# opentrack/neuralnet-tracker-traincode

Hardware: AMD Instinct MI355X
Metric: face-crops/sec fwd+bwd @ batch 512 (higher is better)
Workload: dtype f32; 1 GPU; NetworkWithPointHead(mobilenetv1, point head on, NLL off = training-script defaults): zero_grad + fwd + multi-task loss + bwd + fused clip/Adam step; per_gpu_batch=512, global_batch=512, input=129x129x1 f32, parallelism=dp1

## Files before the change

### neuralnet-tracker-traincode_amd/csrc/pwconv_r.hip

```cpp
#include "ttk_common.h"
#include "conv_geom.h"
#include "split16.h"
#include <type_traits>


namespace ttk {

enum { RMODE_FWD = 0, RMODE_DGRAD = 1 };
template <int N, typename F, int I = 0>
__device__ __forceinline__ void static_for(F&& f) {
  if constexpr (I < N) {
    f(std::integral_constant<int, I>{});
    static_for<N, F, I + 1>(static_cast<F&&>(f));
  }
}
__device__ __forceinline__ f32x16 rmfma(f16x8 a, f16x8 b, f32x16 c) { return __builtin_amdgcn_mfma_f32_32x32x16_f16(a, b, c, 0, 0, 0); }
constexpr int kRBN = 256;

__device__ __forceinline__ void rbarrier() {
  asm volatile("s_waitcnt lgkmcnt(0)" ::: "memory");
  __builtin_amdgcn_s_barrier();
  asm volatile("" ::: "memory");
}

__device__ __forceinline__ unsigned rlow2(unsigned h, float x0, float x1) {
  unsigned l;
  asm("v_fma_mixlo_f16 %0, %1, -1.0, %2 op_sel_hi:[1,0,0]\n\t"
      "v_fma_mixhi_f16 %0, %1, -1.0, %3 op_sel:[1,0,0] op_sel_hi:[1,0,0]"
      : "=&v"(l)
      : "v"(h), "v"(x0), "v"(x1));
  return l;
}
__device__ __forceinline__ __amdgpu_buffer_rsrc_t rbuf(const float* base) {
  return __builtin_amdgcn_make_buffer_rsrc(const_cast<float*>(base), 0, 0x7fffffff, 0x00020000);
}
__device__ __forceinline__ f32x4 rbuf_ld4(__amdgpu_buffer_rsrc_t r, unsigned elem_off) {
  return __builtin_bit_cast(f32x4, __builtin_amdgcn_raw_buffer_load_b128(r, elem_off * 4u, 0, 2));
}

template <int RBLK>
struct RGeo {
  static constexpr int RB = 32 * RBLK;
  static constexpr int WM = RBLK == 8 ? 4 : 2, WN = 8 / WM;
  static constexpr int TM = RBLK / WM, TN = 8 / WN;
  static constexpr int APL = RB * 32, BPL = kRBN * 32;
  static constexpr int kStage = 2 * APL + 2 * BPL;
  static constexpr int kStr = kStage + 64;
  static constexpr int kRing = 2 * 2 * kStr;
  static constexpr int CH = 32 * WM;
  static constexpr int LDC = kRBN + 4;
  static constexpr int kEpi = CH * LDC * 4 + 12 * 2 * kRBN * 4;
  static constexpr int kCst = 4 * 1024 * 4;
  static constexpr int kSmem = kRing + kCst > kEpi ? kRing + kCst : kEpi;
};

template <int RBLK, int MODE, int NW, typename Acc, bool M16 = false>
__device__ __forceinline__ void r_epilogue(unsigned char* lds, Acc& acc, float* __restrict__ out, const float* __restrict__ E0, const float* __restrict__ bnE,
                                           float* __restrict__ part, int64_t M, int Nout, int64_t m0, int64_t m_end, int n0, unsigned by, float sa, float sb) {
  using G = RGeo<RBLK>;
  constexpr int WM = G::WM, WN = G::WN, TM = G::TM, TN = G::TN;
  constexpr bool FWD = MODE == RMODE_FWD;
  const int tid = threadIdx.x;
  const int wave = __builtin_amdgcn_readfirstlane(tid >> 6);
  constexpr int LDC = G::LDC, CH = G::CH;
  float* Cs = reinterpret_cast<float*>(lds);
  float* red = reinterpret_cast<float*>(lds + CH * LDC * 4);
  const int hw_ = tid >> 5, c4 = (hw_ & 7) * 8 + (tid & 7), rg = (hw_ >> 3) * 4 + ((tid >> 3) & 3);
  const int col = n0 + 4 * c4;
  const float inv = 1.f / (sa * sb);
  float4 esc = f4(0.f), emean = f4(0.f), ebeta = f4(0.f);
  if constexpr (!FWD) {
    esc = ld4(bnE + TTK_BN_SCALE * Nout + col); emean = ld4(bnE + TTK_BN_MEAN * Nout + col); ebeta = ld4(bnE + TTK_BN_BETA * Nout + col);
  } else {
    if (bnE) emean = ld4(bnE + col);
  }
  float4 s1 = f4(0.f), s2 = f4(0.f);
  constexpr int NRG = NW == 12 ? 6 : 8, NGRP = (CH + NW * NRG - 1) / (NW * NRG);
  float4 ev[2][NRG];
  auto tile_row = [&](int c, int cr) -> int64_t { return m0 + (cr >> 5) * (32 * TM) + c * 32 + (cr & 31); };
  auto e_load = [&](auto idxc) {
    constexpr int idx = decltype(idxc)::value, c = idx / NGRP, g = idx % NGRP;
    if constexpr (!FWD && idx < TM * NGRP) {
#pragma unroll
      for (int u = 0; u < NRG; ++u) {
        const int cr = rg + NW * (g * NRG + u);
        const int64_t grow = tile_row(c, cr);
        ev[idx & 1][u] = f4(0.f);
        if (cr < CH && grow < m_end) ev[idx & 1][u] = ld4(E0 + act_off(grow, col, M));
      }
    }
  };
  static_for<TM>([&](auto cc) {
    constexpr int c = decltype(cc)::value;
    if (wave < 8) {
      const int lane = tid & 63, wm = wave / WN, wn = wave % WN, r = lane & 31, h = lane >> 5;
      if constexpr (M16) {
        const int r16 = lane & 15, g4 = lane >> 4;
#pragma unroll
        for (int s_ = 0; s_ < 2; ++s_)
#pragma unroll
          for (int j = 0; j < 2 * TN; ++j)
#pragma unroll
            for (int i = 0; i < 4; ++i) Cs[(wm * 32 + s_ * 16 + 4 * g4 + i) * LDC + wn * (32 * TN) + j * 16 + r16] = acc[2 * c + s_][j][i];
      } else {
#pragma unroll
      for (int j = 0; j < TN; ++j)
#pragma unroll
        for (int e = 0; e < 16; ++e) Cs[(wm * 32 + (e & 3) + 8 * (e >> 2) + 4 * h) * LDC + wn * (32 * TN) + j * 32 + r] = acc[c][j][e];
      }
    }
    if constexpr (c == 0) e_load(std::integral_constant<int, 0>{});
    __syncthreads();
    static_for<NGRP>([&](auto gc) {
      constexpr int g = decltype(gc)::value, idx = c * NGRP + g;
      e_load(std::integral_constant<int, idx + 1>{});
#pragma unroll
      for (int u = 0; u < NRG; ++u) {
        const int cr = rg + NW * (g * NRG + u);
        const int64_t grow = tile_row(c, cr);
        if (cr >= CH || grow >= m_end) continue;
        float4 v = ld4(Cs + cr * LDC + 4 * c4);
        v = make_float4(v.x * inv, v.y * inv, v.z * inv, v.w * inv);
        const size_t o = act_off(grow, col, M);
        if constexpr (FWD) {
          st4(out + o, v);
          v = sub4(v, emean);
          s1 = add4(s1, v);
          s2 = fma4(v, v, s2);
        } else {
          const float4 yc = sub4(ev[idx & 1][u], emean);
          v = mask4(v, fma4(esc, yc, ebeta));
          st4(out + o, v);
          s1 = add4(s1, v);
          s2 = fma4(v, yc, s2);
        }
      }
    });
    __syncthreads();
  });
  if (part) {
    st4(red + (rg * 2 + 0) * kRBN + 4 * c4, s1);
    st4(red + (rg * 2 + 1) * kRBN + 4 * c4, s2);
    __syncthreads();
    if (tid < 2 * kRBN) {
      const int which = tid / kRBN, c = tid % kRBN;
      float a = 0.f;
#pragma unroll
      for (int qq = 0; qq < NW; ++qq) a += red[(qq * 2 + which) * kRBN + c];
      part[(size_t)by * 2 * Nout + (size_t)which * Nout + n0 + c] = a;
    }
  }
}

template <int RBLK, int MODE>
__global__ void __launch_bounds__(768) pw16r_k(const float* __restrict__ A0, const float* __restrict__ A1, const float* __restrict__ bnA,
                                               const uint16_t* __restrict__ Bq, const float* __restrict__ wmax, float* __restrict__ out,
                                               const float* __restrict__ E0, const float* __restrict__ bnE, float* __restrict__ part, int64_t M,
                                               int K, int Nout, int RT) {
  using G = RGeo<RBLK>;
  constexpr int RB = G::RB, WM = G::WM, WN = G::WN, TM = G::TM, TN = G::TN, APL = G::APL, BPL = G::BPL, kStr = G::kStr;
  constexpr bool FWD = MODE == RMODE_FWD;
  __shared__ __attribute__((aligned(16))) unsigned char lds[G::kSmem];

  const int tid = threadIdx.x;
  const unsigned Gd = gridDim.x, Lid = blockIdx.x, NB = Nout / kRBN;
  const unsigned xq = Gd / 8, xr = Gd % 8, xcd = Lid % 8;
  const unsigned tile = (xcd < xr ? xcd * (xq + 1) : xr * (xq + 1) + (xcd - xr) * xq) + Lid / 8;
  const unsigned bx = tile % NB, by = tile / NB;
  const int64_t m0 = (int64_t)by * RT;
  const int64_t m_end = m0 + RT < M ? m0 + RT : M;
  const int n0 = bx * kRBN;
  const int nks = K / 32;
  const int wave = __builtin_amdgcn_readfirstlane(tid >> 6);
  const float sa = pow2_scale(bnA[(size_t)TTK_BN_AUX * K + (FWD ? TTK_AUX_ACT_BOUND : TTK_AUX_DY_BOUND)]);
  const float sb = pow2_scale(*wmax);
  f32x16 acc[TM][TN];
  float* cst = reinterpret_cast<float*>(lds + G::kRing);
  {
    constexpr int NQ = FWD ? 3 : 4;
    for (int i = tid * 4; i < NQ * K; i += 768 * 4) {
      const int j = i / K, c = i - j * K;
      const int row = FWD ? (j == 0 ? TTK_BN_SCALE : (j == 1 ? TTK_BN_MEAN : TTK_BN_BETA)) : (j == 0 ? TTK_BN_GA : (j == 1 ? TTK_BN_GMEAN : (j == 2 ? TTK_BN_GB : TTK_BN_MEAN)));
      float4 v = ld4(bnA + (size_t)row * K + c);
      if (j == 0 || j == 2) v = make_float4(v.x * sa, v.y * sa, v.z * sa, v.w * sa);
      st4(cst + i, v);
    }
    __syncthreads();
  }

  if (wave >= 8) {
    __builtin_amdgcn_s_setprio(3);
    const int pt = tid - 512;
    const int row0 = pt >> 3, kq8 = pt & 7;
    const int sub = kq8 >> 2, chunk = (kq8 >> 1) & 1, o8 = (kq8 & 1) * 8;
    constexpr int AP = RBLK;
    constexpr int GPS = FWD ? 1 : 2;
    constexpr int NSLOT = FWD ? 2 : 3;
    static_assert(AP % GPS == 0 && (GPS & (GPS - 1)) == 0, "groups per step: a power of two that divides the row passes");
    constexpr int G = AP / GPS;
    constexpr int UNR = NSLOT % GPS == 0 ? NSLOT : (GPS % NSLOT == 0 ? GPS : NSLOT * GPS);
    f32x4 ra0[NSLOT][G] = {}, ra1[NSLOT][FWD ? 1 : G] = {};
    unsigned live = 0u;
#pragma unroll
    for (int i = 0; i < AP; ++i) live |= (m0 + row0 + 32 * i < m_end ? 1u : 0u) << i;
    const unsigned aoff0 = (unsigned)(row0 * kCB + kq8 * 4);
    const float* cq = cst + kq8 * 4;
    unsigned char* wbase = lds + sub * kStr + o8;
    const int NG = nks * GPS;

    auto load_g = [&](int ks, auto hfc, auto slotc) {
      constexpr int slot = decltype(slotc)::value, hf = decltype(hfc)::value;
      const __amdgpu_buffer_rsrc_t r0 = rbuf(A0 + ((size_t)ks * act_block_stride(M) + (size_t)m0 * kCB));
      const __amdgpu_buffer_rsrc_t r1 = rbuf((FWD ? (const float*)nullptr : A1) + ((size_t)ks * act_block_stride(M) + (size_t)m0 * kCB));
#pragma unroll
      for (int u = 0; u < G; ++u) {
        const int i = hf * G + u;
        const unsigned o = ((live >> i) & 1u) ? aoff0 + (unsigned)(i * 32 * kCB) : (unsigned)(kq8 * 4);
        ra0[slot][u] = rbuf_ld4(r0, o);
        if constexpr (!FWD) ra1[slot][u] = rbuf_ld4(r1, o);
      }
    };
    auto conv_g = [&](int ks, auto hfc, auto slotc) {
      constexpr int slot = decltype(slotc)::value, hf = decltype(hfc)::value;
      unsigned char* S = wbase + (ks & 1) * 2 * kStr;
      const float* cs = cq + ks * 32;
      const f32x4 c0 = *reinterpret_cast<const f32x4*>(cs), q1 = *reinterpret_cast<const f32x4*>(cs + K), c2 = *reinterpret_cast<const f32x4*>(cs + 2 * K);
      f32x4 q3 = c2;
      if constexpr (!FWD) q3 = *reinterpret_cast<const f32x4*>(cs + 3 * K);
#pragma unroll
      for (int u = 0; u < G; ++u) {
        const int i = hf * G + u;
        f32x4 v;
        if constexpr (FWD) {
          v = c0 * (ra0[slot][u] - q1) + c2;
          v.x = fmaxf(v.x, 0.f); v.y = fmaxf(v.y, 0.f); v.z = fmaxf(v.z, 0.f); v.w = fmaxf(v.w, 0.f);
        } else {
          v = c0 * (ra0[slot][u] - q1) + c2 * (ra1[slot][u] - q3);
        }
        if (!((live >> i) & 1u)) v = f32x4{0.f, 0.f, 0.f, 0.f};
        split_store16(v, S + swz16(row0 + 32 * i, chunk), APL);
      }
    };
    static_for<NSLOT>([&](auto dc) {
      constexpr int d = decltype(dc)::value;
      if (d < NG) load_g(d / GPS, std::integral_constant<int, d % GPS>{}, dc);
    });
    for (int n0 = 0; n0 < NG; n0 += UNR) {
      static_for<UNR>([&](auto dc) {
        constexpr int d = decltype(dc)::value;
        using HF = std::integral_constant<int, d % GPS>;
        using SL = std::integral_constant<int, d % NSLOT>;
        const int n = n0 + d;
        if (n < NG) {
          conv_g(n / GPS, HF{}, SL{});
          if (n + NSLOT < NG) load_g((n + NSLOT) / GPS, std::integral_constant<int, (d + NSLOT) % GPS>{}, SL{});
          if constexpr (d % GPS == GPS - 1) {
            __builtin_amdgcn_sched_barrier(0);
            rbarrier();
          }
        }
      });
    }
    rbarrier();
  } else {
    const int lane = tid & 63, wm = wave / WN, wn = wave % WN;
    const int r = lane & 31, h = lane >> 5;
    constexpr bool HOLD_A = TM <= TN;
    constexpr int TH = HOLD_A ? TM : TN, TS = HOLD_A ? TN : TM;
    constexpr int HPL = HOLD_A ? APL : BPL, SPL = HOLD_A ? BPL : APL;
    int hold_off[TH], strm_off[TS];
#pragma unroll
    for (int x = 0; x < TH; ++x) hold_off[x] = HOLD_A ? swz16(wm * (32 * TM) + x * 32 + r, h) : 2 * APL + swz16(wn * (32 * TN) + x * 32 + r, h);
#pragma unroll
    for (int x = 0; x < TS; ++x) strm_off[x] = HOLD_A ? 2 * APL + swz16(wn * (32 * TN) + x * 32 + r, h) : swz16(wm * (32 * TM) + x * 32 + r, h);
#pragma unroll
    for (int i = 0; i < TM; ++i)
#pragma unroll
      for (int j = 0; j < TN; ++j)
#pragma unroll
        for (int e = 0; e < 16; ++e) acc[i][j][e] = 0.f;
    f16x8 hold[TH][2] = {}, strm[2][2] = {};
    const int64_t bplane = (int64_t)K * Nout;
    const uint16_t* bsrc = Bq + ((wave >> 1) & 1) * bplane + ((int64_t)(wave >> 2) * Nout + n0 + (wave & 1) * 128) * 16 + lane * 8;
    const int bdst = (wave >> 2) * kStr + 2 * APL + ((wave >> 1) & 1) * BPL + (wave & 1) * 4096;
    const unsigned lds_base = (unsigned)(size_t)(__attribute__((address_space(3))) unsigned char*)lds;
    auto dma_b = [&](int ks) {
      const uint16_t* sp = bsrc + (int64_t)ks * 2 * Nout * 16;
      const unsigned d = __builtin_amdgcn_readfirstlane(lds_base + (unsigned)((ks & 1) * 2 * kStr + bdst));
#pragma unroll
      for (int j = 0; j < 4; ++j) {
        unsigned keep;
        asm volatile("s_mov_b32 %0, m0\n\ts_mov_b32 m0, %2\n\ts_nop 0\n\tglobal_load_lds_dwordx4 %1, off\n\ts_mov_b32 m0, %0"
                     : "=&s"(keep)
                     : "v"(sp + j * 512), "s"(d + j * 1024)
                     : "memory");
      }
    };
    dma_b(0);
    asm volatile("s_waitcnt vmcnt(0)" ::: "memory");
    rbarrier();
    auto rd = [&](const unsigned char* S, int plane_bytes, int off, int p) { return *reinterpret_cast<const f16x8*>(S + p * plane_bytes + off); };
    for (int it = 0; it < nks; ++it) {
      if (it + 1 < nks) dma_b(it + 1);
      const unsigned char* S0 = lds + (it & 1) * 2 * kStr;
#pragma unroll
      for (int p = 0; p < 2; ++p) {
#pragma unroll
        for (int y = 0; y < TH; ++y) hold[y][p] = rd(S0, HPL, hold_off[y], p);
        strm[0][p] = rd(S0, SPL, strm_off[0], p);
      }
#pragma unroll
      for (int sub = 0; sub < 2; ++sub) {
        const unsigned char* S = S0 + sub * kStr;
#pragma unroll
        for (int x = 0; x < TS; ++x) {
          const int cur = (sub * TS + x) & 1;
          const bool last = x + 1 == TS;
          if (!last) {
#pragma unroll
            for (int p = 0; p < 2; ++p) strm[cur ^ 1][p] = rd(S, SPL, strm_off[x + 1], p);
          } else if (sub == 0) {
#pragma unroll
            for (int p = 0; p < 2; ++p) strm[cur ^ 1][p] = rd(S + kStr, SPL, strm_off[0], p);
          }
#pragma unroll
          for (int y = 0; y < TH; ++y) {
            if constexpr (HOLD_A) {
              acc[y][x] = rmfma(hold[y][0], strm[cur][1], acc[y][x]);
              acc[y][x] = rmfma(hold[y][1], strm[cur][0], acc[y][x]);
              acc[y][x] = rmfma(hold[y][0], strm[cur][0], acc[y][x]);
            } else {
              acc[x][y] = rmfma(strm[cur][0], hold[y][1], acc[x][y]);
              acc[x][y] = rmfma(strm[cur][1], hold[y][0], acc[x][y]);
              acc[x][y] = rmfma(strm[cur][0], hold[y][0], acc[x][y]);
            }
            if (last && sub == 0) {
#pragma unroll
              for (int p = 0; p < 2; ++p) hold[y][p] = rd(S + kStr, HPL, hold_off[y], p);
            }
          }
        }
      }
      asm volatile("s_waitcnt vmcnt(0)" ::: "memory");
      rbarrier();
    }
  }
  r_epilogue<RBLK, MODE, 12>(lds, acc, out, E0, bnE, part, M, Nout, m0, m_end, n0, by, sa, sb);
}

template <int RBLK>
struct MGeo {
  using G = RGeo<RBLK>;
  static constexpr int NW = 8;
  static constexpr int kEpi = G::CH * G::LDC * 4 + NW * 2 * kRBN * 4;
  static constexpr int kSmem = G::kRing + G::kCst > kEpi ? G::kRing + G::kCst : kEpi;
};

template <int RBLK>
__global__ void __launch_bounds__(512) pw16m_k(const float* __restrict__ A0, const float* __restrict__ A1, const float* __restrict__ bnA,
                                               const uint16_t* __restrict__ Bq, const float* __restrict__ wmax, float* __restrict__ out,
                                               const float* __restrict__ E0, const float* __restrict__ bnE, float* __restrict__ part, int64_t M,
                                               int K, int Nout, int RT) {
  using G = RGeo<RBLK>;
  constexpr int RB = G::RB, WM = G::WM, WN = G::WN, TM = G::TM, TN = G::TN, APL = G::APL, BPL = G::BPL, kStr = G::kStr;
  __shared__ __attribute__((aligned(16))) unsigned char lds[MGeo<RBLK>::kSmem];

  const int tid = threadIdx.x;
  const unsigned Gd = gridDim.x, Lid = blockIdx.x, NB = Nout / kRBN;
  const unsigned xq = Gd / 8, xr = Gd % 8, xcd = Lid % 8;
  const unsigned tile = (xcd < xr ? xcd * (xq + 1) : xr * (xq + 1) + (xcd - xr) * xq) + Lid / 8;
  const unsigned bx = tile % NB, by = tile / NB;
  const int64_t m0 = (int64_t)by * RT;
  const int64_t m_end = m0 + RT < M ? m0 + RT : M;
  const int n0 = bx * kRBN;
  const int nks = K / 32;
  const int wave = __builtin_amdgcn_readfirstlane(tid >> 6);
  const float sa = pow2_scale(bnA[(size_t)TTK_BN_AUX * K + TTK_AUX_DY_BOUND]);
  const float sb = pow2_scale(*wmax);
  f32x4 acc16[2 * TM][2 * TN];
  float* cst = reinterpret_cast<float*>(lds + G::kRing);
  {
    for (int i = tid * 4; i < 4 * K; i += 512 * 4) {
      const int j = i / K, c = i - j * K;
      const int row = j == 0 ? TTK_BN_GA : (j == 1 ? TTK_BN_GMEAN : (j == 2 ? TTK_BN_GB : TTK_BN_MEAN));
      float4 v = ld4(bnA + (size_t)row * K + c);
      if (j == 0 || j == 2) v = make_float4(v.x * sa, v.y * sa, v.z * sa, v.w * sa);
      st4(cst + i, v);
    }
    __syncthreads();
  }

  const int row0 = tid >> 3, kq8 = tid & 7;
  const int sub_ = kq8 >> 2, chunk = (kq8 >> 1) & 1, o8 = (kq8 & 1) * 8;
  constexpr int AP = RB / 64;
  constexpr int NA = AP * 2;
  f32x4 ra0[2][AP] = {}, ra1[2][AP] = {};
  unsigned live = 0u;
#pragma unroll
  for (int u = 0; u < AP; ++u) live |= (m0 + row0 + 64 * u < m_end ? 1u : 0u) << u;
  const unsigned aoff0 = (unsigned)(row0 * kCB + kq8 * 4);
  const float* cq = cst + kq8 * 4;
  unsigned char* wbase = lds + sub_ * kStr + o8 + swz16(row0, chunk);

  auto load_a = [&](int ks, auto setc) {
    constexpr int set = decltype(setc)::value;
    const __amdgpu_buffer_rsrc_t r0 = rbuf(A0 + ((size_t)ks * act_block_stride(M) + (size_t)m0 * kCB));
    const __amdgpu_buffer_rsrc_t r1 = rbuf(A1 + ((size_t)ks * act_block_stride(M) + (size_t)m0 * kCB));
#pragma unroll
    for (int u = 0; u < AP; ++u) {
      const unsigned o = ((live >> u) & 1u) ? aoff0 + (unsigned)(u * 64 * kCB) : (unsigned)(kq8 * 4);
      ra0[set][u] = rbuf_ld4(r0, o);
      ra1[set][u] = rbuf_ld4(r1, o);
    }
  };
  f32x4 cc0 = {}, cq1 = {}, cc2 = {}, cq3 = {};
  f32x4 pv = {};
  uint2 ph = make_uint2(0u, 0u);
  auto conv_consts = [&](int ks) {
    const float* cs = cq + ks * 32;
    cc0 = *reinterpret_cast<const f32x4*>(cs); cq1 = *reinterpret_cast<const f32x4*>(cs + K); cc2 = *reinterpret_cast<const f32x4*>(cs + 2 * K);
    cq3 = *reinterpret_cast<const f32x4*>(cs + 3 * K);
  };
  int conv_ks = 0;
  auto conv_part = [&](auto setc, auto slotc, auto ppc) {
    constexpr int set = decltype(setc)::value, slot = decltype(slotc)::value, pp = decltype(ppc)::value, u = pp >> 1;
    if constexpr ((pp & 1) == 0) {
      conv_consts(conv_ks);
      f32x4 v = cc0 * (ra0[set][u] - cq1) + cc2 * (ra1[set][u] - cq3);
      if (m0 + 64 * u + 63 >= m_end) {
        if (!((live >> u) & 1u)) v = f32x4{0.f, 0.f, 0.f, 0.f};
      }
      const f16x2 h01 = __builtin_convertvector(f32x2{v.x, v.y}, f16x2), h23 = __builtin_convertvector(f32x2{v.z, v.w}, f16x2);
      pv = v;
      ph = make_uint2(__builtin_bit_cast(unsigned, h01), __builtin_bit_cast(unsigned, h23));
    } else {
      const unsigned l01 = rlow2(ph.x, pv.x, pv.y), l23 = rlow2(ph.y, pv.z, pv.w);
      unsigned char* dst = wbase + slot * 2 * kStr + u * 64 * 32;
      *reinterpret_cast<uint2*>(dst) = ph;
      *reinterpret_cast<uint2*>(dst + APL) = make_uint2(l01, l23);
    }
  };

  const int lane = tid & 63, wm = wave / WN, wn = wave % WN;
  static_assert(TM * TN == RBLK && 2 * AP == RBLK, "4 RBLK MFMA triples per step, one of the 2 AP conversion parts behind every fourth");
  const int r = lane & 31, h = lane >> 5;
  constexpr bool HOLD_A = TM <= TN;
  constexpr int TH = HOLD_A ? TM : TN;
  int hold_off[TH];
#pragma unroll
  for (int x = 0; x < TH; ++x) hold_off[x] = HOLD_A ? swz16(wm * (32 * TM) + x * 32 + r, h) : 2 * APL + swz16(wn * (32 * TN) + x * 32 + r, h);
#pragma unroll
  for (int i = 0; i < 2 * TM; ++i)
#pragma unroll
    for (int j = 0; j < 2 * TN; ++j) acc16[i][j] = f32x4{0.f, 0.f, 0.f, 0.f};
  int a16_off[2 * TM], b16_off[2 * TN];
  const int live_rows16 = (int)(m_end - m0) - wm * (32 * TM);
  const int r16 = lane & 15, g4 = lane >> 4;
#pragma unroll
  for (int i = 0; i < 2 * TM; ++i) a16_off[i] = (g4 >> 1) * kStr + swz16(wm * (32 * TM) + i * 16 + r16, g4 & 1);
#pragma unroll
  for (int j = 0; j < 2 * TN; ++j) b16_off[j] = (g4 >> 1) * kStr + 2 * APL + swz16(wn * (32 * TN) + j * 16 + r16, g4 & 1);
  const int64_t bplane = (int64_t)K * Nout;
  const uint16_t* bsrc = Bq + ((wave >> 1) & 1) * bplane + ((int64_t)(wave >> 2) * Nout + n0 + (wave & 1) * 128) * 16 + lane * 8;
  const int bdst = (wave >> 2) * kStr + 2 * APL + ((wave >> 1) & 1) * BPL + (wave & 1) * 4096;
  const unsigned lds_base = (unsigned)(size_t)(__attribute__((address_space(3))) unsigned char*)lds;
  auto dma_b = [&](int ks, int slot) {
    const uint16_t* sp = bsrc + (int64_t)ks * 2 * Nout * 16;
    const unsigned d = __builtin_amdgcn_readfirstlane(lds_base + (unsigned)(slot * 2 * kStr + bdst));
#pragma unroll
    for (int j = 0; j < 4; ++j) {
      unsigned keep;
      asm volatile("s_mov_b32 %0, m0\n\ts_mov_b32 m0, %2\n\ts_nop 0\n\tglobal_load_lds_dwordx4 %1, off\n\ts_mov_b32 m0, %0"
                   : "=&s"(keep)
                   : "v"(sp + j * 512), "s"(d + j * 1024)
                   : "memory");
    }
  };
  auto rd = [&](const unsigned char* S, int plane_bytes, int off, int p) { return *reinterpret_cast<const f16x8*>(S + p * plane_bytes + off); };
  using P0 = std::integral_constant<int, 0>;
  using P1 = std::integral_constant<int, 1>;

  load_a(0, P0{});
  if (nks > 1) load_a(1, P1{});
  dma_b(0, 0);
  conv_consts(0);
  conv_ks = 0;
  static_for<RBLK>([&](auto ppc) { conv_part(P0{}, P0{}, ppc); });
  if (nks > 2) {
    load_a(2, P0{});
    asm volatile("s_waitcnt vmcnt(%0)" ::"n"(NA) : "memory");
  } else {
    asm volatile("s_waitcnt vmcnt(0)" ::: "memory");
  }
  rbarrier();

  auto step = [&](int it, auto parc, auto convc) {
    constexpr int PAR = decltype(parc)::value;
    constexpr bool CONV = decltype(convc)::value != 0;
    using SN = std::integral_constant<int, PAR ^ 1>;
    const unsigned char* S0 = lds + PAR * 2 * kStr;
    if constexpr (CONV) {
      dma_b(it + 1, PAR ^ 1);
      conv_ks = it + 1;
    }
    f16x8 hb[2 * TN][2], sa16[2][2];
#pragma unroll
    for (int p = 0; p < 2; ++p) {
#pragma unroll
      for (int j = 0; j < 2 * TN; ++j) hb[j][p] = rd(S0, BPL, b16_off[j], p);
      sa16[0][p] = rd(S0, APL, a16_off[0], p);
    }
    static_for<2 * TM>([&](auto ic) {
      constexpr int i = decltype(ic)::value, cur = i & 1;
      if constexpr (i + 1 < 2 * TM) {
#pragma unroll
        for (int p = 0; p < 2; ++p) sa16[cur ^ 1][p] = rd(S0, APL, a16_off[i + 1], p);
      }
      const bool blk_live = i * 16 < live_rows16;
      static_for<2 * TN>([&](auto jc) {
        constexpr int j = decltype(jc)::value;
        if (blk_live) {
          acc16[i][j] = __builtin_amdgcn_mfma_f32_16x16x32_f16(sa16[cur][0], hb[j][1], acc16[i][j], 0, 0, 0);
          acc16[i][j] = __builtin_amdgcn_mfma_f32_16x16x32_f16(sa16[cur][1], hb[j][0], acc16[i][j], 0, 0, 0);
          acc16[i][j] = __builtin_amdgcn_mfma_f32_16x16x32_f16(sa16[cur][0], hb[j][0], acc16[i][j], 0, 0, 0);
        }
        constexpr int q = i * (2 * TN) + j;
        if constexpr (CONV && (q & 3) == 3) {
          conv_part(SN{}, SN{}, std::integral_constant<int, (q >> 2)>{});
          __builtin_amdgcn_sched_barrier(0);
        }
      });
    });
    if constexpr (CONV) {
      if (it + 3 < nks) {
        load_a(it + 3, SN{});
        asm volatile("s_waitcnt vmcnt(%0)" ::"n"(NA) : "memory");
      } else {
        asm volatile("s_waitcnt vmcnt(0)" ::: "memory");
      }
    }
    rbarrier();
  };
  int it = 0;
  for (; it + 2 < nks; it += 2) {
    step(it, P0{}, P1{});
    step(it + 1, P1{}, P1{});
  }
  if (it + 1 < nks) {
    step(it, P0{}, P1{});
    step(it + 1, P1{}, P0{});
  } else {
    step(it, P0{}, P0{});
  }
  r_epilogue<RBLK, RMODE_DGRAD, 8, decltype(acc16), true>(lds, acc16, out, E0, bnE, part, M, Nout, m0, m_end, n0, by, sa, sb);
}

constexpr int kTRow = 576;
constexpr int kTPlane = 16 * kTRow;
constexpr int kTStage = 4 * kTPlane;
constexpr int kTRing = 2 * 2 * kTStage;

__device__ __forceinline__ f16x8 tr_frag(const unsigned char* plane, int off) {
  const s16x4 lo = __builtin_amdgcn_ds_read_tr16_b64_v4i16((__attribute__((address_space(3))) s16x4*)(plane + off));
  const s16x4 hi = __builtin_amdgcn_ds_read_tr16_b64_v4i16((__attribute__((address_space(3))) s16x4*)(plane + off + 4 * kTRow));
  const s16x8 v = __builtin_shufflevector(lo, hi, 0, 1, 2, 3, 4, 5, 6, 7);
  return __builtin_bit_cast(f16x8, v);
}
__device__ __forceinline__ void tsplit_store(f32x4 v, unsigned char* dst) { split_store16(v, dst, kTPlane); }

__global__ void __launch_bounds__(768) pw16u_wgrad_k(const float* __restrict__ G, const float* __restrict__ Y, const float* __restrict__ bn_pw,
                                                     const float* __restrict__ X, const float* __restrict__ bn_x, float* __restrict__ partial,
                                                     int64_t M, int Cin, int Cout, int64_t rows_per_slice) {
  __shared__ __attribute__((aligned(16))) unsigned char lds[kTRing];
  const int tid = threadIdx.x;
  const unsigned NT = (Cout / 128) * (Cin / 256), NG = gridDim.x, Lid = blockIdx.x;
  const unsigned xq = NG / 8, xr = NG % 8, xcd = Lid % 8;
  const unsigned logical = (xcd < xr ? xcd * (xq + 1) : xr * (xq + 1) + (xcd - xr) * xq) + Lid / 8;
  const unsigned tile = logical % NT, slice = logical / NT;
  const int tiles_k = Cin / 256;
  const int n0 = (tile / tiles_k) * 128, k0 = (tile % tiles_k) * 256;
  const int64_t m_begin = (int64_t)slice * rows_per_slice;
  const int64_t m_end = (m_begin + rows_per_slice < M) ? m_begin + rows_per_slice : M;
  const int nks = m_begin < m_end ? (int)((m_end - m_begin + 31) / 32) : 0;
  const int wave = __builtin_amdgcn_readfirstlane(tid >> 6);
  const float sa = pow2_scale(bn_pw[(size_t)TTK_BN_AUX * Cout + TTK_AUX_DY_BOUND]);
  const float sb = pow2_scale(bn_x[(size_t)TTK_BN_AUX * Cin + TTK_AUX_ACT_BOUND]);

  if (wave >= 4) {
    __builtin_amdgcn_s_setprio(3);
    const int pw = wave - 4, lane = tid & 63;
    const int qa = lane & 31, ra = 2 * (lane >> 5);
    const int ca = n0 + 4 * qa, cb = k0 + 4 * lane;
    const f32x4 ga = *reinterpret_cast<const f32x4*>(bn_pw + TTK_BN_GA * Cout + ca) * sa;
    const f32x4 gb = *reinterpret_cast<const f32x4*>(bn_pw + TTK_BN_GB * Cout + ca) * sa;
    const f32x4 gmean = *reinterpret_cast<const f32x4*>(bn_pw + TTK_BN_GMEAN * Cout + ca);
    const f32x4 ymean = *reinterpret_cast<const f32x4*>(bn_pw + TTK_BN_MEAN * Cout + ca);
    const f32x4 sc = *reinterpret_cast<const f32x4*>(bn_x + TTK_BN_SCALE * Cin + cb) * sb;
    const f32x4 mu = *reinterpret_cast<const f32x4*>(bn_x + TTK_BN_MEAN * Cin + cb);
    const f32x4 be = *reinterpret_cast<const f32x4*>(bn_x + TTK_BN_BETA * Cin + cb) * sb;
    f32x4 rg[2][2], ry[2][2], rx[2][4];
    const int64_t r0 = m_begin + 4 * pw;
    const size_t oa = act_off(0, ca, M), ob = act_off(0, cb, M);
    unsigned char* wbase = lds + (pw >> 2) * kTStage + (4 * (pw & 3)) * kTRow;
    unsigned char* wdy = wbase + ra * kTRow + qa * 8;
    unsigned char* wx = wbase + 2 * kTPlane + lane * 8;
    auto load = [&](int ks, auto setc) {
      constexpr int set = decltype(setc)::value;
      const int64_t rb = r0 + (int64_t)ks * 32;
#pragma unroll
      for (int i = 0; i < 4; ++i) {
        int64_t row = rb + i;
        row = row < m_end ? row : m_end - 1;
        rx[set][i] = ld_act4(X + ob + (size_t)row * kCB);
      }
#pragma unroll
      for (int j = 0; j < 2; ++j) {
        int64_t row = rb + ra + j;
        row = row < m_end ? row : m_end - 1;
        rg[set][j] = ld_act4(G + oa + (size_t)row * kCB);
        ry[set][j] = ld_act4(Y + oa + (size_t)row * kCB);
      }
    };
    auto store = [&](int ks, auto setc) {
      constexpr int set = decltype(setc)::value;
      unsigned char* dy = wdy + (ks & 1) * 2 * kTStage;
      unsigned char* xx = wx + (ks & 1) * 2 * kTStage;
      const int64_t rb = r0 + (int64_t)ks * 32;
#pragma unroll
      for (int j = 0; j < 2; ++j) {
        f32x4 v = ga * (rg[set][j] - gmean) + gb * (ry[set][j] - ymean);
        if (!(rb + ra + j < m_end)) v = f32x4{0.f, 0.f, 0.f, 0.f};
        tsplit_store(v, dy + j * kTRow);
      }
#pragma unroll
      for (int i = 0; i < 4; ++i) {
        f32x4 a = sc * (rx[set][i] - mu) + be;
        a.x = fmaxf(a.x, 0.f); a.y = fmaxf(a.y, 0.f); a.z = fmaxf(a.z, 0.f); a.w = fmaxf(a.w, 0.f);
        if (!(rb + i < m_end)) a = f32x4{0.f, 0.f, 0.f, 0.f};
        tsplit_store(a, xx + i * kTRow);
      }
    };
    using S0 = std::integral_constant<int, 0>;
    using S1 = std::integral_constant<int, 1>;
    if (nks > 0) {
      load(0, S0{});
      if (nks > 1) load(1, S1{});
      for (int s = 0; s < nks; s += 2) {
        store(s, S0{});
        if (s + 2 < nks) load(s + 2, S0{});
        rbarrier();
        if (s + 1 < nks) {
          store(s + 1, S1{});
          if (s + 3 < nks) load(s + 3, S1{});
          rbarrier();
        }
      }
      rbarrier();
    }
  } else {
    f32x16 acc[2][4];
    const int lane = tid & 63, wm = wave >> 1, wn = wave & 1;
    const int grp = lane >> 4, q = (lane & 15) >> 2, p4 = lane & 3, h = grp >> 1;
    const int lane_off = (8 * h + q) * kTRow + (16 * (grp & 1) + 4 * p4) * 2;
    int aoff[2], boff[4];
#pragma unroll
    for (int i = 0; i < 2; ++i) aoff[i] = lane_off + (wm * 64 + i * 32) * 2;
#pragma unroll
    for (int j = 0; j < 4; ++j) boff[j] = 2 * kTPlane + lane_off + (wn * 128 + j * 32) * 2;
#pragma unroll
    for (int i = 0; i < 2; ++i)
#pragma unroll
      for (int j = 0; j < 4; ++j)
#pragma unroll
        for (int e = 0; e < 16; ++e) acc[i][j][e] = 0.f;
    if (nks > 0) {
      rbarrier();
      for (int it = 0; it < nks; ++it) {
#pragma unroll
        for (int sub = 0; sub < 2; ++sub) {
          const unsigned char* S = lds + ((it & 1) * 2 + sub) * kTStage;
          f16x8 a[2][2], b[2][2];
#pragma unroll
          for (int pl = 0; pl < 2; ++pl) {
#pragma unroll
            for (int i = 0; i < 2; ++i) a[i][pl] = tr_frag(S + pl * kTPlane, aoff[i]);
            b[0][pl] = tr_frag(S + pl * kTPlane, boff[0]);
          }
#pragma unroll
          for (int j = 0; j < 4; ++j) {
            const int cur = j & 1;
            if (j + 1 < 4) {
#pragma unroll
              for (int pl = 0; pl < 2; ++pl) b[cur ^ 1][pl] = tr_frag(S + pl * kTPlane, boff[j + 1]);
            }
#pragma unroll
            for (int i = 0; i < 2; ++i) {
              acc[i][j] = __builtin_amdgcn_mfma_f32_32x32x16_f16(a[i][0], b[cur][1], acc[i][j], 0, 0, 0);
              acc[i][j] = __builtin_amdgcn_mfma_f32_32x32x16_f16(a[i][1], b[cur][0], acc[i][j], 0, 0, 0);
              acc[i][j] = __builtin_amdgcn_mfma_f32_32x32x16_f16(a[i][0], b[cur][0], acc[i][j], 0, 0, 0);
            }
          }
        }
        rbarrier();
      }
    }
    const float inv = 1.f / (sa * sb);
    const int r = lane & 31, hh = lane >> 5;
    float* dst = partial + (size_t)slice * Cout * Cin;
#pragma unroll
    for (int i = 0; i < 2; ++i)
#pragma unroll
      for (int j = 0; j < 4; ++j)
#pragma unroll
        for (int e = 0; e < 16; ++e) {
          const int row = n0 + wm * 64 + i * 32 + (e & 3) + 8 * (e >> 2) + 4 * hh;
          const int col = k0 + wn * 128 + j * 32 + r;
          dst[(size_t)row * Cin + col] = acc[i][j][e] * inv;
        }
  }
}

__global__ void __launch_bounds__(256) wgrad_fold_k(const float* __restrict__ partial, float* __restrict__ dW, int64_t n, int slices) {
  const int64_t i = ((int64_t)blockIdx.x * 256 + threadIdx.x) * 4;
  if (i >= n) return;
  float4 a = ld4(dW + i);
  int s = 0;
  for (; s + 8 <= slices; s += 8) {
    float4 v[8];
#pragma unroll
    for (int u = 0; u < 8; ++u) v[u] = ld4nt(partial + (size_t)(s + u) * n + i);
#pragma unroll
    for (int u = 0; u < 8; ++u) a = add4(a, v[u]);
  }
  for (; s < slices; ++s) a = add4(a, ld4nt(partial + (size_t)s * n + i));
  st4(dW + i, a);
}

bool f16t_wgrad_shape(int Cin, int Cout) {
  if (Cin < 256 || Cin % 256) return false;
  return Cout >= 128 && Cout % 128 == 0 && !(Cin == 256 && Cout == 256);
}
static void t_wgrad_plan(int64_t M, int Cin, int Cout, int& tiles, int64_t& slices, int64_t& rows) {
  tiles = (Cout / 128) * (Cin / 256);
  slices = 256 / tiles;
  if (slices < 1) slices = 1;
  const int64_t max_slices = ceil_div(M, 64);
  if (slices > max_slices) slices = max_slices;
  rows = ceil_div(ceil_div(M, slices), 32) * 32;
  slices = ceil_div(M, rows);
}
size_t f16t_wgrad_scratch_bytes(int64_t M, int Cin, int Cout) {
  if (!f16t_wgrad_shape(Cin, Cout)) return 0;
  int tiles;
  int64_t slices, rows;
  t_wgrad_plan(M, Cin, Cout, tiles, slices, rows);
  return (size_t)slices * Cin * Cout * sizeof(float);
}
bool launch_f16t_wgrad(const float* g, const float* y, const float* bn_pw, const float* ydw, const float* bn_dw, float* dw, float* partial, int64_t M,
                       int Cin, int Cout, hipStream_t st) {
  if (!partial || !f16t_wgrad_shape(Cin, Cout)) return false;
  int tiles;
  int64_t slices, rows;
  t_wgrad_plan(M, Cin, Cout, tiles, slices, rows);
  hipLaunchKernelGGL(pw16u_wgrad_k, dim3((unsigned)(tiles * slices)), dim3(768), 0, st, g, y, bn_pw, ydw, bn_dw, partial, M, Cin, Cout, rows);
  const int64_t n = (int64_t)Cin * Cout;
  hipLaunchKernelGGL(wgrad_fold_k, dim3((unsigned)ceil_div(n, 1024)), dim3(256), 0, st, partial, dw, n, (int)slices);
  return true;
}

bool f16r_gemm_shape(int K, int Nout, int dgrad) {
  if (K < 128 || K > 1024 || K % 32 != 0 || Nout < 256 || Nout % kRBN != 0) return false;
  return !(dgrad && K == 256 && Nout == 256);
}

struct RPlan { int rblk, rt, row_blocks; };
static RPlan r_plan(int64_t M, int K, int Nout) {
  static const int cus = [] { int dev = 0, n = 256; if (hipGetDevice(&dev) == hipSuccess) (void)hipDeviceGetAttribute(&n, hipDeviceAttributeMultiprocessorCount, dev); return n > 0 ? n : 256; }();
  const int ct = Nout / kRBN, steps = K / 32;
  RPlan best{0, 0, 0};
  double best_cost = 1e300;
  for (int rblk = 4; rblk <= 8; rblk += 2) {
    const int RB = 32 * rblk;
    for (int r = 1; r <= 4096; ++r) {
      const int64_t rb = (int64_t)cus * r / ct;
      if (rb < 1) continue;
      int64_t rt = ceil_div(M, rb);
      if (rt > RB) continue;
      if (rt < 32) rt = 32;
      const int64_t row_blocks = ceil_div(M, rt);
      const double tiles = (double)row_blocks * ct, rounds = (double)ceil_div((int64_t)tiles, cus);
      const double step = fmax(384.0 * rblk, rt * 128.0 / 12.0 + 32768.0 / 35.0);
      const double cost = rounds * (steps * step + rt * 1024.0 / 10.0 + 3000.0);
      if (cost < best_cost) { best_cost = cost; best = RPlan{rblk, (int)rt, (int)row_blocks}; }
      break;
    }
  }
  if (best.rblk == 0)
    best = RPlan{8, 256, (int)ceil_div(M, 256)};
  return best;
}
int f16r_partial_rows(int64_t M, int K, int Nout, int dgrad) { return f16r_gemm_shape(K, Nout, dgrad) ? r_plan(M, K, Nout).row_blocks : 0; }
int f16r_tile_rows(int64_t M, int K, int Nout, int dgrad) { return f16r_gemm_shape(K, Nout, dgrad) ? 32 * r_plan(M, K, Nout).rblk : 0; }

__global__ void w16r_split_k(const float* __restrict__ w, uint16_t* __restrict__ q, const float* __restrict__ wmax, int rows, int K) {
  const int64_t n = (int64_t)rows * K;
  const int64_t i = (int64_t)blockIdx.x * blockDim.x + threadIdx.x;
  if (i >= n) return;
  const float s = pow2_scale(*wmax);
  const int row = (int)(i / K), k = (int)(i - (int64_t)row * K);
  const int64_t o = r_plane_index(row, k, rows);
  uint16_t h, l;
  split16(w[i] * s, h, l);
  q[o] = h;
  q[n + o] = l;
}

template <int MODE>
bool launch_f16r_gemm(const float* A0, const float* A1, const float* bnA, const float* Bm, float* out, const float* E0, const float* bnE, float* part,
                      int64_t M, int K, int Nout, void* planes, float* wmax, hipStream_t st) {
  if (!planes || !wmax || !f16r_gemm_shape(K, Nout, MODE == RMODE_DGRAD)) return false;
  uint16_t* Bq = reinterpret_cast<uint16_t*>(planes);
  const int64_t nw = (int64_t)Nout * K;
  if (Bm) {
    launch_w16_absmax(Bm, nw, wmax, st);
    hipLaunchKernelGGL(w16r_split_k, dim3((unsigned)ceil_div(nw, 256)), dim3(256), 0, st, Bm, Bq, wmax, Nout, K);
  }
  const RPlan pl = r_plan(M, K, Nout);
  const unsigned tiles = (unsigned)pl.row_blocks * (Nout / kRBN);
#define TTK_M_LAUNCH(RBLK_) \
  hipLaunchKernelGGL((pw16m_k<RBLK_>), dim3(tiles), dim3(512), 0, st, A0, A1, bnA, Bq, wmax, out, E0, bnE, part, M, K, Nout, pl.rt)
#define TTK_R_LAUNCH(RBLK_) \
  hipLaunchKernelGGL((pw16r_k<RBLK_, MODE>), dim3(tiles), dim3(768), 0, st, A0, A1, bnA, Bq, wmax, out, E0, bnE, part, M, K, Nout, pl.rt)
  if constexpr (MODE == RMODE_DGRAD) {
    if (pl.rblk == 4) TTK_M_LAUNCH(4);
    else if (pl.rblk == 6) TTK_M_LAUNCH(6);
    else TTK_R_LAUNCH(8);
  } else {
    if (pl.rblk == 4) TTK_R_LAUNCH(4);
    else if (pl.rblk == 6) TTK_R_LAUNCH(6);
    else TTK_R_LAUNCH(8);
  }
#undef TTK_R_LAUNCH
#undef TTK_M_LAUNCH
  return true;
}

template bool launch_f16r_gemm<RMODE_FWD>(const float*, const float*, const float*, const float*, float*, const float*, const float*, float*, int64_t,
                                          int, int, void*, float*, hipStream_t);
template bool launch_f16r_gemm<RMODE_DGRAD>(const float*, const float*, const float*, const float*, float*, const float*, const float*, float*, int64_t,
                                            int, int, void*, float*, hipStream_t);

}
```

Baseline: 72280 crops/s.

## Switch pointwise-conv main loop to 16x16x32 MFMA with tail-row skipping

Replaces the 32x32x16 f16 MFMA accumulation in the consumer waves of the fused pointwise conv kernel with 16x16x32 MFMA tiles, restructuring LDS operand reads and register blocking around 16-row fragments. It also adds a compile-time specialised k-loop that skips MFMAs for 16-row blocks beyond the live rows of a partial tile. The intent is finer-grained work skipping on ragged M tails and a different issue/latency balance. The cost is a changed accumulator layout that the epilogue must handle (passed as a new template parameter), plus more LDS reads and instructions per tile.

```diff
diff --git a/neuralnet-tracker-traincode_amd/csrc/pwconv_r.hip b/neuralnet-tracker-traincode_amd/csrc/pwconv_r.hip
--- a/neuralnet-tracker-traincode_amd/csrc/pwconv_r.hip
+++ b/neuralnet-tracker-traincode_amd/csrc/pwconv_r.hip
@@ -14,7 +14,6 @@
     static_for<N, F, I + 1>(static_cast<F&&>(f));
   }
 }
-__device__ __forceinline__ f32x16 rmfma(f16x8 a, f16x8 b, f32x16 c) { return __builtin_amdgcn_mfma_f32_32x32x16_f16(a, b, c, 0, 0, 0); }
 constexpr int kRBN = 256;
 
 __device__ __forceinline__ void rbarrier() {
@@ -174,7 +173,7 @@
   const int wave = __builtin_amdgcn_readfirstlane(tid >> 6);
   const float sa = pow2_scale(bnA[(size_t)TTK_BN_AUX * K + (FWD ? TTK_AUX_ACT_BOUND : TTK_AUX_DY_BOUND)]);
   const float sb = pow2_scale(*wmax);
-  f32x16 acc[TM][TN];
+  f32x4 acc[2 * TM][2 * TN];
   float* cst = reinterpret_cast<float*>(lds + G::kRing);
   {
     constexpr int NQ = FWD ? 3 : 4;
@@ -264,22 +263,7 @@
     rbarrier();
   } else {
     const int lane = tid & 63, wm = wave / WN, wn = wave % WN;
-    const int r = lane & 31, h = lane >> 5;
-    constexpr bool HOLD_A = TM <= TN;
-    constexpr int TH = HOLD_A ? TM : TN, TS = HOLD_A ? TN : TM;
-    constexpr int HPL = HOLD_A ? APL : BPL, SPL = HOLD_A ? BPL : APL;
-    int hold_off[TH], strm_off[TS];
-#pragma unroll
-    for (int x = 0; x < TH; ++x) hold_off[x] = HOLD_A ? swz16(wm * (32 * TM) + x * 32 + r, h) : 2 * APL + swz16(wn * (32 * TN) + x * 32 + r, h);
-#pragma unroll
-    for (int x = 0; x < TS; ++x) strm_off[x] = HOLD_A ? 2 * APL + swz16(wn * (32 * TN) + x * 32 + r, h) : swz16(wm * (32 * TM) + x * 32 + r, h);
-#pragma unroll
-    for (int i = 0; i < TM; ++i)
-#pragma unroll
-      for (int j = 0; j < TN; ++j)
-#pragma unroll
-        for (int e = 0; e < 16; ++e) acc[i][j][e] = 0.f;
-    f16x8 hold[TH][2] = {}, strm[2][2] = {};
+    const int live_rows = (int)(m_end - m0) - wm * (32 * TM);
     const int64_t bplane = (int64_t)K * Nout;
     const uint16_t* bsrc = Bq + ((wave >> 1) & 1) * bplane + ((int64_t)(wave >> 2) * Nout + n0 + (wave & 1) * 128) * 16 + lane * 8;
     const int bdst = (wave >> 2) * kStr + 2 * APL + ((wave >> 1) & 1) * BPL + (wave & 1) * 4096;
@@ -300,52 +284,89 @@
     asm volatile("s_waitcnt vmcnt(0)" ::: "memory");
     rbarrier();
     auto rd = [&](const unsigned char* S, int plane_bytes, int off, int p) { return *reinterpret_cast<const f16x8*>(S + p * plane_bytes + off); };
-    for (int it = 0; it < nks; ++it) {
-      if (it + 1 < nks) dma_b(it + 1);
-      const unsigned char* S0 = lds + (it & 1) * 2 * kStr;
-#pragma unroll
-      for (int p = 0; p < 2; ++p) {
-#pragma unroll
-        for (int y = 0; y < TH; ++y) hold[y][p] = rd(S0, HPL, hold_off[y], p);
-        strm[0][p] = rd(S0, SPL, strm_off[0], p);
-      }
-#pragma unroll
-      for (int sub = 0; sub < 2; ++sub) {
-        const unsigned char* S = S0 + sub * kStr;
-#pragma unroll
-        for (int x = 0; x < TS; ++x) {
-          const int cur = (sub * TS + x) & 1;
-          const bool last = x + 1 == TS;
-          if (!last) {
-#pragma unroll
-            for (int p = 0; p < 2; ++p) strm[cur ^ 1][p] = rd(S, SPL, strm_off[x + 1], p);
-          } else if (sub == 0) {
-#pragma unroll
-            for (int p = 0; p < 2; ++p) strm[cur ^ 1][p] = rd(S + kStr, SPL, strm_off[0], p);
+    const int r16 = lane & 15, g4 = lane >> 4;
+    const int a16_off = (g4 >> 1) * kStr + swz16(wm * (32 * TM) + r16, g4 & 1);
+    const int b16_off = (g4 >> 1) * kStr + 2 * APL + swz16(wn * (32 * TN) + r16, g4 & 1);
+    constexpr int kBlk16 = 16 * 32;
+#pragma unroll
+    for (int i = 0; i < 2 * TM; ++i)
+#pragma unroll
+      for (int j = 0; j < 2 * TN; ++j) acc[i][j] = f32x4{0.f, 0.f, 0.f, 0.f};
+    auto mfma3 = [&](f32x4& c, const f16x8 (&a)[2], const f16x8 (&b)[2]) {
+      c = __builtin_amdgcn_mfma_f32_16x16x32_f16(a[0], b[1], c, 0, 0, 0);
+      c = __builtin_amdgcn_mfma_f32_16x16x32_f16(a[1], b[0], c, 0, 0, 0);
+      c = __builtin_amdgcn_mfma_f32_16x16x32_f16(a[0], b[0], c, 0, 0, 0);
+    };
+    auto k_loop = [&](auto fullc) {
+      constexpr bool FULL = decltype(fullc)::value != 0;
+      for (int it = 0; it < nks; ++it) {
+        if (it + 1 < nks) dma_b(it + 1);
+        const unsigned char* S0 = lds + (it & 1) * 2 * kStr;
+        if constexpr (RBLK < 8) {
+          f16x8 hb[2 * TN][2], sa16[2][2];
+#pragma unroll
+          for (int p = 0; p < 2; ++p) {
+#pragma unroll
+            for (int j = 0; j < 2 * TN; ++j) hb[j][p] = rd(S0, BPL, b16_off + j * kBlk16, p);
+            sa16[0][p] = rd(S0, APL, a16_off, p);
           }
-#pragma unroll
-          for (int y = 0; y < TH; ++y) {
-            if constexpr (HOLD_A) {
-              acc[y][x] = rmfma(hold[y][0], strm[cur][1], acc[y][x]);
-              acc[y][x] = rmfma(hold[y][1], strm[cur][0], acc[y][x]);
-              acc[y][x] = rmfma(hold[y][0], strm[cur][0], acc[y][x]);
-            } else {
-              acc[x][y] = rmfma(strm[cur][0], hold[y][1], acc[x][y]);
-              acc[x][y] = rmfma(strm[cur][1], hold[y][0], acc[x][y]);
-              acc[x][y] = rmfma(strm[cur][0], hold[y][0], acc[x][y]);
+          static_for<2 * TM>([&](auto ic) {
+            constexpr int i = decltype(ic)::value, cur = i & 1;
+            if constexpr (i + 1 < 2 * TM) {
+#pragma unroll
+              for (int p = 0; p < 2; ++p) sa16[cur ^ 1][p] = rd(S0, APL, a16_off + (i + 1) * kBlk16, p);
             }
-            if (last && sub == 0) {
-#pragma unroll
-              for (int p = 0; p < 2; ++p) hold[y][p] = rd(S + kStr, HPL, hold_off[y], p);
+            if (FULL || i * 16 < live_rows) {
+#pragma unroll
+              for (int j = 0; j < 2 * TN; ++j) mfma3(acc[i][j], sa16[cur], hb[j]);
             }
+          });
+        } else {
+          f16x8 ha[TM][2], sb[2];
+#pragma unroll
+          for (int p = 0; p < 2; ++p) {
+#pragma unroll
+            for (int y = 0; y < TM; ++y) ha[y][p] = rd(S0, APL, a16_off + y * kBlk16, p);
+            sb[p] = rd(S0, BPL, b16_off, p);
           }
+          static_for<2>([&](auto hc) {
+            constexpr int half = decltype(hc)::value;
+            static_for<2 * TN>([&](auto jc) {
+              constexpr int j = decltype(jc)::value;
+              constexpr bool last = j + 1 == 2 * TN, more = !last || half == 0;
+              constexpr int nxt = (last ? 0 : j + 1) * kBlk16;
+#pragma unroll
+              for (int y = 0; y < TM; ++y) {
+                f32x4& c = acc[half * TM + y][j];
+                if (FULL || (half * TM + y) * 16 < live_rows) c = __builtin_amdgcn_mfma_f32_16x16x32_f16(ha[y][0], sb[1], c, 0, 0, 0);
+              }
+              if constexpr (more) sb[1] = rd(S0, BPL, b16_off + nxt, 1);
+              __builtin_amdgcn_sched_barrier(0);
+#pragma unroll
+              for (int y = 0; y < TM; ++y) {
+                f32x4& c = acc[half * TM + y][j];
+                if (FULL || (half * TM + y) * 16 < live_rows) {
+                  c = __builtin_amdgcn_mfma_f32_16x16x32_f16(ha[y][1], sb[0], c, 0, 0, 0);
+                  c = __builtin_amdgcn_mfma_f32_16x16x32_f16(ha[y][0], sb[0], c, 0, 0, 0);
+                }
+                if constexpr (last && half == 0) {
+#pragma unroll
+                  for (int p = 0; p < 2; ++p) ha[y][p] = rd(S0, APL, a16_off + (TM + y) * kBlk16, p);
+                }
+              }
+              if constexpr (more) sb[0] = rd(S0, BPL, b16_off + nxt, 0);
+              __builtin_amdgcn_sched_barrier(0);
+            });
+          });
         }
-      }
-      asm volatile("s_waitcnt vmcnt(0)" ::: "memory");
-      rbarrier();
-    }
-  }
-  r_epilogue<RBLK, MODE, 12>(lds, acc, out, E0, bnE, part, M, Nout, m0, m_end, n0, by, sa, sb);
+        asm volatile("s_waitcnt vmcnt(0)" ::: "memory");
+        rbarrier();
+      }
+    };
+    if (live_rows >= 32 * TM) k_loop(std::integral_constant<int, 1>{});
+    else k_loop(std::integral_constant<int, 0>{});
+  }
+  r_epilogue<RBLK, MODE, 12, decltype(acc), true>(lds, acc, out, E0, bnE, part, M, Nout, m0, m_end, n0, by, sa, sb);
 }
 
 template <int RBLK>
```

Result: no change. 72720 crops/s, median of 6 (+0.6%).
